# HarryShomer/LPFormer

Hardware: AMD Instinct MI355X
Metric: candidate link-pairs scored/sec (whole node) (higher is better)
Workload: dtype f32

## Files before the change

### lpformer_amd/csrc/tail_chain.hip

```cpp
#include <type_traits>

#include "lpf_common.h"

namespace {

typedef float f32x4 __attribute__((ext_vector_type(4)));

#ifndef LPF_TC_GROUPS
#define LPF_TC_GROUPS 4
#endif
constexpr int TC_GROUPS = LPF_TC_GROUPS;
constexpr int TC_WAVES = 2 * TC_GROUPS;
constexpr int TC_THREADS = 64 * TC_WAVES;

struct TailArgs {
    int64_t M;
    const float *x; int64_t ldx; int KA;
    const float *addend; int64_t ldadd;
    const float *wA, *lnA_g, *lnA_b; int NA;
    const float *tail; int64_t ldtail;
    const float *wB, *bB, *lnB_g, *lnB_b; int NB;
    const float *re; int64_t ldre;
    const float *wC, *bC; int NC;
    const float *wdot, *bdot;
    float *logit, *prob;
    const float *part;
    const float *bnd;
    int64_t units_cap;
    const int32_t *type_ptr;
    const float *att_bias;
    const int64_t *sel_ctl;
    int n_counts;
    const float *rows; int64_t ldrows;
    const int32_t *perm;
    const int64_t *n_full;
    const float *bC_empty;
    const float *row_empty;
    const float *X; int64_t ldX;
    const int64_t *batch; int64_t batch_ld, n_rows;
    const float *wE, *bE, *lnE_g, *lnE_b;
};

constexpr int tc_per_thread(int ntp) { return (ntp * 64 + TC_THREADS - 1) / TC_THREADS; }
constexpr int tc_stage_stride(int ntp) { return (ntp * 64 + 511) / 512 * 512; }

typedef short bf16x4_bits __attribute__((ext_vector_type(4)));
template <int P, int NTP, typename T>
__device__ __forceinline__ void tc_load(T (&r)[P], const float *packed, int stage, int tid) {
    const T *src = reinterpret_cast<const T *>(packed) + (int64_t)stage * tc_stage_stride(NTP);
#pragma unroll
    for (int e = 0; e < P; ++e) {
        const int i = e * TC_THREADS + tid;
#ifdef TC_NOWLOAD
        r[e] = T{};
        (void)src; (void)i;
#else
        r[e] = src[i < tc_stage_stride(NTP) ? i : 0];
#endif
    }
}
template <int P, typename T>
__device__ __forceinline__ void tc_store(const T (&r)[P], T *slab, int tid) {
#pragma unroll
    for (int e = 0; e < P; ++e) slab[e * TC_THREADS + tid] = r[e];
}

#define TC_PIN() __builtin_amdgcn_sched_barrier(0)

template <int TPW>
__device__ __forceinline__ void tc_mfma(f32x4 (&acc)[TPW], const f32x4 *lw, const f32x4 bv, bool last = true) {
    f32x4 a[TPW];
#pragma unroll
    for (int c = 0; c < TPW; ++c) a[c] = lw[c * 64];
#pragma unroll
    for (int u = 0; u < 4; ++u) {
#pragma unroll
        for (int c = 0; c < TPW - 1; ++c) acc[c] = __builtin_amdgcn_mfma_f32_16x16x4f32(a[c][u], bv[u], acc[c], 0, 0, 0);
        if (last) acc[TPW - 1] = __builtin_amdgcn_mfma_f32_16x16x4f32(a[TPW - 1][u], bv[u], acc[TPW - 1], 0, 0, 0);
    }
}
template <int TPW>
__device__ __forceinline__ void tc_mfma(f32x4 (&acc)[TPW], const uint2 *lw, const f32x4 bv, bool last = true) {
    bf16x4_bits b;
#pragma unroll
    for (int u = 0; u < 4; ++u) b[u] = (short)lpf_f32_to_bf16(bv[u]);
#pragma unroll
    for (int c = 0; c < TPW; ++c) {
        if (c == TPW - 1 && !last) break;
        const uint2 w = lw[c * 64];
        const bf16x4_bits a = {(short)(w.x & 0xffffu), (short)(w.x >> 16), (short)(w.y & 0xffffu), (short)(w.y >> 16)};
        acc[c] = __builtin_amdgcn_mfma_f32_16x16x16bf16_1k(a, b, acc[c], 0, 0, 0);
    }
}

constexpr int TC_XCH_SLOT = TC_WAVES * 16;
template <int TPW>
__device__ __forceinline__ void tc_layernorm(f32x4 (&acc)[TPW], int fbase, int n, const float *g, const float *b, int half,
                                             int q, float *my_x, const float *peer_x, bool relu) {
    float s1 = 0.f;
#pragma unroll
    for (int c = 0; c < TPW; ++c) s1 += acc[c][0] + acc[c][1] + acc[c][2] + acc[c][3];
    s1 = lpf_quad_sum(s1);
    if (q == 0) *my_x = s1;
    __syncthreads();
    const float mean = (half == 0 ? s1 + *peer_x : *peer_x + s1) / (float)n;
    float s2 = 0.f;
#pragma unroll
    for (int c = 0; c < TPW; ++c)
#pragma unroll
        for (int r = 0; r < 4; ++r) {
            const float d = (fbase + 16 * c + r < n) ? acc[c][r] - mean : 0.f;
            s2 += d * d;
        }
    s2 = lpf_quad_sum(s2);
    if (q == 0) my_x[TC_XCH_SLOT] = s2;
    __syncthreads();
    const float p2 = peer_x[TC_XCH_SLOT];
    const float rstd = 1.0f / sqrtf((half == 0 ? s2 + p2 : p2 + s2) / (float)n + 1e-5f);
#pragma unroll
    for (int c = 0; c < TPW; ++c) {
        const f32x4 gg = *reinterpret_cast<const f32x4 *>(g + fbase + 16 * c);
        const f32x4 bb = *reinterpret_cast<const f32x4 *>(b + fbase + 16 * c);
        acc[c] = (acc[c] - mean) * rstd * gg + bb;
        if (relu) {
#pragma unroll
            for (int r = 0; r < 4; ++r) acc[c][r] = fmaxf(acc[c][r], 0.f);
        }
    }
}

#ifdef TC_STAMPS
__device__ uint64_t *tc_stamp_buf = nullptr;
#define TC_STAMP(k) do { if (lane == 0) st_t[k] = wall_clock64(); } while (0)
#define TC_STAMPS_OUT(kind) do { if (lane == 0 && tc_stamp_buf) { uint64_t *o__ = tc_stamp_buf + ((int64_t)blockIdx.x * TC_WAVES + wave) * 16; \
        for (int k__ = 0; k__ < 10; ++k__) o__[k__] = st_t[k__]; o__[15] = (kind); } } while (0)
#define TC_STAMP_ROWS() do { __builtin_amdgcn_s_waitcnt(0x0f70); TC_STAMP(8); } while (0)
#else
#define TC_STAMP_ROWS() do { } while (0)
#define TC_STAMP(k) do { } while (0)
#define TC_STAMPS_OUT(kind) do { } while (0)
#endif

template <int NTA, int NTB, int NTC>
struct TcShape {
    static constexpr int NTPA = (NTA + 1) & ~1, NTPB = (NTB + 1) & ~1, NTPC = (NTC + 1) & ~1;
    static constexpr int PA = tc_per_thread(NTPA), PB = tc_per_thread(NTPB), PC = tc_per_thread(NTPC);
    static constexpr int PM = PA > PB ? (PA > PC ? PA : PC) : (PB > PC ? PB : PC);
    static constexpr int SLAB = PM * TC_THREADS;
    static constexpr int HT = NTPA > NTPB ? NTPA : NTPB;
    static constexpr int HID = TC_GROUPS * HT * 64;
    static constexpr int XCH = 5 * TC_WAVES * 16;
    static constexpr int VEC_B = 3 * 16 * NTPA, VEC_C = VEC_B + 3 * 16 * NTPB, VEC_N = VEC_C + 2 * 16 * NTPC;
    static constexpr size_t BYTES = (size_t)(2 * SLAB + HID) * sizeof(f32x4) + (XCH + VEC_N) * sizeof(float);
    static_assert(NTC >= 32 || BYTES <= 81920, "two workgroups share a CU's 160 KB of LDS");
};

template <int NTA, int NTB, int NTC, int WM = 0, bool ROWS = false, bool EW = false>
__global__ __launch_bounds__(TC_THREADS, NTC >= 32 ? 2 : (TC_THREADS >= 512 ? 4 : 3)) void tail_chain_kernel(const TailArgs A) {
    using S = TcShape<NTA, NTB, NTC>;
    constexpr bool WB = WM != 0;
    using WT = typename std::conditional<WM == 1, uint2, f32x4>::type;
    constexpr int NTPA = S::NTPA, NTPB = S::NTPB, NTPC = S::NTPC;
    constexpr int TPWA = NTPA / 2, TPWB = NTPB / 2, TPWC = NTPC / 2;
    constexpr int NGE = NTA;
    extern __shared__ __attribute__((aligned(16))) f32x4 lds[];
    f32x4 *hid = lds + 2 * S::SLAB;
    float *xch = reinterpret_cast<float *>(hid + S::HID);
    const int tid = threadIdx.x, lane = tid & 63, wave = tid >> 6;
    const int grp = wave >> 1, half = wave & 1, q = lane >> 4, j = lane & 15;
    float *my_x = xch + wave * 16 + j;
    const float *peer_x = xch + (wave ^ 1) * 16 + j;
    float *vec = xch + S::XCH;
    f32x4 *my_hid = hid + (grp * S::HT) * 64 + lane;
    int buf = 0;
#ifdef TC_STAMPS
    uint64_t st_t[10] = {0};
    TC_STAMP(0);
#endif

    const int64_t tile = blockIdx.x;
    const int64_t pos = tile * (16 * TC_GROUPS) + grp * 16 + j;
    const bool live = pos < A.M;
    bool lite = false;
    int64_t m = pos;
    if constexpr (ROWS) {
        if (A.perm) {
            m = A.perm[live ? pos : A.M - 1];
            lite = tile * (16 * TC_GROUPS) >= *A.n_full;
        }
    }
    const int64_t mm = live ? m : (ROWS && A.perm ? m : A.M - 1);
    bool no_sel = false;
    if constexpr (ROWS) no_sel = A.perm && A.row_empty && (live ? pos : A.M - 1) >= *A.n_full;

    constexpr int VP0 = EW ? 0 : S::VEC_B / 4, VPN = S::VEC_N / 4 - VP0, VPT = (VPN + TC_THREADS - 1) / TC_THREADS;
    f32x4 vecr[VPT];
#pragma unroll
    for (int e = 0; e < VPT; ++e) {
        int p = VP0 + e * TC_THREADS + tid;
        p = p < S::VEC_N / 4 ? p : S::VEC_N / 4 - 1;
        const float *src;
        if (p >= S::VEC_C / 4) {
            const int o = p - S::VEC_C / 4;
            src = o < 4 * NTPC ? (lite ? A.bC_empty : A.bC) + 4 * o : A.wdot + 4 * (o - 4 * NTPC);
        } else if (!EW || p >= S::VEC_B / 4) {
            const int o = p - S::VEC_B / 4;
            src = o < 4 * NTPB ? A.bB + 4 * o : (o < 8 * NTPB ? A.lnB_g + 4 * (o - 4 * NTPB) : A.lnB_b + 4 * (o - 8 * NTPB));
        } else {
            src = p < 4 * NTPA ? A.bE + 4 * p : (p < 8 * NTPA ? A.lnE_g + 4 * (p - 4 * NTPA) : A.lnE_b + 4 * (p - 8 * NTPA));
        }
        vecr[e] = *reinterpret_cast<const f32x4 *>(src);
    }
    TC_PIN();
    auto tc_vec_publish = [&]() __attribute__((always_inline)) {
#pragma unroll
        for (int e = 0; e < VPT; ++e) {
            int p = VP0 + e * TC_THREADS + tid;
            p = p < S::VEC_N / 4 ? p : S::VEC_N / 4 - 1;
            reinterpret_cast<f32x4 *>(vec)[p] = vecr[e];
        }
    };
    const float *v_bE = vec, *v_lnE_g = vec + 16 * NTPA, *v_lnE_b = vec + 32 * NTPA;
    const float *v_bB = vec + S::VEC_B, *v_lnB_g = v_bB + 16 * NTPB, *v_lnB_b = v_bB + 32 * NTPB;
    const float *v_bC = vec + S::VEC_C, *v_wdot = v_bC + 16 * NTPC;

    f32x4 rowv[ROWS ? TPWA : 1], rowt = (f32x4){0.f, 0.f, 0.f, 0.f};
#pragma unroll
    for (int c = 0; c < (ROWS ? TPWA : 1); ++c) rowv[c] = (f32x4){0.f, 0.f, 0.f, 0.f};
    auto tc_rows_request = [&]() __attribute__((always_inline)) {
        if constexpr (ROWS) {
            const int fbase = 16 * half * TPWA + 4 * q;
            const float *own = A.rows + mm * A.ldrows, *row = no_sel ? A.row_empty : own;
#pragma unroll
            for (int c = 0; c < TPWA; ++c) {
                const int f0 = fbase + 16 * c;
                rowv[c] = *reinterpret_cast<const f32x4 *>(row + (f0 < A.NA ? f0 : 0));
            }
            rowt = *reinterpret_cast<const f32x4 *>(own + A.NA);
        }
    };

    f32x4 accC[TPWC];
    if constexpr (EW) {
        static_assert(ROWS && WM == 0 && S::PA == 1 && NTPA == NTA && NGE % 2 == 0 && 2 * tc_stage_stride(NTPA) <= S::SLAB &&
                          tc_stage_stride(2 * NTPA) == 2 * tc_stage_stride(NTPA), "stage E: the fp32 rows form at D = 128");
        constexpr int TE_KG = 68, TE_Q2 = 34;
        static_assert((NGE - 1) * TE_KG + TE_Q2 + 32 <= S::HT * 64, "stage E's product tiles fit a group's hidden tiles");
        const int gj = 8 * half + (lane >> 3), gp = lane & 7;
        const int64_t gpos = tile * (16 * TC_GROUPS) + grp * 16 + gj;
        const int64_t gm = gpos < A.M ? gpos : A.M - 1;
        const int64_t gmm = A.perm ? A.perm[gm] : gm;
        int64_t ra = A.batch[gmm], rb = A.batch[A.batch_ld + gmm];
        WT wrE[2];
        tc_load<2, 2 * NTPA>(wrE, A.wE, 0, tid);
        TC_PIN();
        if ((uint64_t)ra >= (uint64_t)A.n_rows) ra = 0;
        if ((uint64_t)rb >= (uint64_t)A.n_rows) rb = 0;
        const float *xa = A.X + ra * A.ldX + 4 * gp, *xb = A.X + rb * A.ldX + 4 * gp;
        f32x4 accE[TPWA];
#pragma unroll
        for (int c = 0; c < TPWA; ++c) accE[c] = (f32x4){0.f, 0.f, 0.f, 0.f};
        f32x4 xra[NGE / 2], xrb[NGE / 2];
#pragma unroll
        for (int i = 0; i < NGE / 2; ++i) {
            xra[i] = *reinterpret_cast<const f32x4 *>(xa + 32 * i);
            xrb[i] = *reinterpret_cast<const f32x4 *>(xb + 32 * i);
        }
        tc_vec_publish();
        TC_STAMP_ROWS();
        {
            f32x4 *pe = hid + (grp * S::HT) * 64 + (gp >> 2) * TE_KG + ((gp >> 1) & 1) * TE_Q2 + (gp & 1) * 16 + gj;
#pragma unroll
            for (int i = 0; i < NGE / 2; ++i) pe[2 * i * TE_KG] = xra[i] * xrb[i];
        }
        const f32x4 *my_pe = hid + (grp * S::HT) * 64 + (q >> 1) * TE_Q2 + (q & 1) * 16 + j;
#pragma unroll
        for (int kg = 0; kg < NGE; kg += 2) {
            WT *lw = reinterpret_cast<WT *>(lds) + buf * S::SLAB;
            tc_store<2>(wrE, lw, tid);
            __syncthreads();
            if (kg + 2 < NGE) tc_load<2, 2 * NTPA>(wrE, A.wE, kg / 2 + 1, tid);
            TC_PIN();
            const f32x4 bv0 = my_pe[kg * TE_KG], bv1 = my_pe[(kg + 1) * TE_KG];
            tc_mfma<TPWA>(accE, lw + (half * TPWA) * 64 + lane, bv0);
            tc_mfma<TPWA>(accE, lw + tc_stage_stride(NTPA) + (half * TPWA) * 64 + lane, bv1);
            TC_PIN();
            buf ^= 1;
        }
        TC_STAMP(9);
        if (!lite) tc_rows_request();
        WT wrCe[S::PC];
        tc_load<S::PC, NTPC>(wrCe, A.wC, 0, tid);
        {
            const int fbase = 16 * half * TPWA + 4 * q;
#pragma unroll
            for (int c = 0; c < TPWA; ++c) accE[c] += *reinterpret_cast<const f32x4 *>(v_bE + fbase + 16 * c);
            tc_layernorm<TPWA>(accE, fbase, A.NA, v_lnE_g, v_lnE_b, half, q, my_x, peer_x, true);
#pragma unroll
            for (int c = 0; c < TPWA; ++c) my_hid[(half * TPWA + c) * 64] = accE[c];
        }
        TC_STAMP(7);
#pragma unroll
        for (int c = 0; c < TPWC; ++c) accC[c] = (f32x4){0.f, 0.f, 0.f, 0.f};
#pragma unroll 1
        for (int kg = 0; kg < NGE; ++kg) {
            WT *lw = reinterpret_cast<WT *>(lds) + buf * S::SLAB;
            tc_store<S::PC>(wrCe, lw, tid);
            __syncthreads();
            if (kg + 1 < NGE) tc_load<S::PC, NTPC>(wrCe, A.wC, kg + 1, tid);
            tc_mfma<TPWC>(accC, lw + (half * TPWC) * 64 + lane, my_hid[kg * 64]);
            buf ^= 1;
        }
        TC_STAMP(4);
        if (!lite) __syncthreads();
    }

    if constexpr (ROWS) {
        if (lite) {
            f32x4 (&acc)[TPWC] = accC;
            if constexpr (!EW) {
#pragma unroll
            for (int c = 0; c < TPWC; ++c) acc[c] = (f32x4){0.f, 0.f, 0.f, 0.f};
            WT wr[S::PC];
            const float *rer = A.re + mm * A.ldre + 4 * q;
            tc_load<S::PC, NTPC>(wr, A.wC, 0, tid);
            f32x4 xr = *reinterpret_cast<const f32x4 *>(rer);
            tc_vec_publish();
#pragma unroll 1
            for (int kg = 0; kg < NGE; ++kg) {
                const f32x4 bv = xr;
                WT *lw = reinterpret_cast<WT *>(lds) + buf * S::SLAB;
                tc_store<S::PC>(wr, lw, tid);
                __syncthreads();
                if (kg + 1 < NGE) {
                    tc_load<S::PC, NTPC>(wr, A.wC, kg + 1, tid);
                    xr = *reinterpret_cast<const f32x4 *>(rer + 16 * (kg + 1));
                }
                tc_mfma<TPWC>(acc, lw + (half * TPWC) * 64 + lane, bv);
                buf ^= 1;
            }
            }
            const int fbase = 16 * half * TPWC + 4 * q;
            float d = 0.f;
#pragma unroll
            for (int c = 0; c < TPWC; ++c) {
                const f32x4 b = *reinterpret_cast<const f32x4 *>(v_bC + fbase + 16 * c);
                const f32x4 w = *reinterpret_cast<const f32x4 *>(v_wdot + fbase + 16 * c);
#pragma unroll
                for (int r = 0; r < 4; ++r) d = fmaf(fmaxf(acc[c][r] + b[r], 0.f), w[r], d);
            }
            d = lpf_quad_sum(d);
            if (q == 0) my_x[4 * TC_XCH_SLOT] = d;
            __syncthreads();
            if (live && q == 0 && half == 0) {
                d = d + peer_x[4 * TC_XCH_SLOT] + A.bdot[0];
                if (A.sel_ctl && A.sel_ctl[3] != 0) d = __builtin_nanf("");
                if (A.logit) A.logit[m] = d;
                if (A.prob) A.prob[m] = 1.0f / (1.0f + expf(-d));
            }
            TC_STAMP(6);
            TC_STAMPS_OUT(1);
            return;
        }
    }
    if constexpr (!EW) tc_vec_publish();
    f32x4 accA[TPWA];
#pragma unroll
    for (int c = 0; c < TPWA; ++c) accA[c] = (f32x4){0.f, 0.f, 0.f, 0.f};
    int seg_cnt[3] = {0, 0, 0};
    if (!WB && !ROWS && A.part == nullptr) {
        const float *xa = A.x + mm * A.ldx;
        const int ngA = (A.KA + 15) >> 4;
        f32x4 wr[S::PA];
        tc_load<S::PA, NTPA>(wr, A.wA, 0, tid);
        int kk = 4 * q < A.KA ? 4 * q : A.KA - 4;
        f32x4 xr = *reinterpret_cast<const f32x4 *>(xa + kk);
#pragma unroll 1
        for (int kg = 0; kg < ngA; ++kg) {
            const f32x4 bv = (16 * kg + 4 * q < A.KA) ? xr : (f32x4){0.f, 0.f, 0.f, 0.f};
            f32x4 *lw = lds + buf * S::SLAB;
            tc_store<S::PA>(wr, lw, tid);
            __syncthreads();
            if (kg + 1 < ngA) {
                tc_load<S::PA, NTPA>(wr, A.wA, kg + 1, tid);
                kk = 16 * (kg + 1) + 4 * q;
                kk = kk < A.KA ? kk : A.KA - 4;
                xr = *reinterpret_cast<const f32x4 *>(xa + kk);
            }
            tc_mfma<TPWA>(accA, lw + (half * TPWA) * 64 + lane, bv);
            buf ^= 1;
        }
    }
    WT wrB[S::PB];
    tc_load<S::PB, NTPB>(wrB, A.wB, 0, tid);
    if constexpr (ROWS) {
        const int fbase = 16 * half * TPWA + 4 * q;
        if constexpr (!EW) tc_rows_request();
#pragma unroll
        for (int c = 0; c < TPWA; ++c) accA[c] = fbase + 16 * c < A.NA ? rowv[c] : (f32x4){0.f, 0.f, 0.f, 0.f};
    } else if (A.part == nullptr) {
        const int fbase = 16 * half * TPWA + 4 * q;
        f32x4 ad[TPWA];
#pragma unroll
        for (int c = 0; c < TPWA; ++c) {
            const int f0 = fbase + 16 * c;
            ad[c] = *reinterpret_cast<const f32x4 *>(A.addend + mm * A.ldadd + (f0 < A.NA ? f0 : 0));
        }
#pragma unroll
        for (int c = 0; c < TPWA; ++c) accA[c] += (fbase + 16 * c < A.NA) ? ad[c] : (f32x4){0.f, 0.f, 0.f, 0.f};
    } else {
        const int fbase = 16 * half * TPWA + 4 * q;
        const int64_t rs = A.NA + 4;
        float mx = -INFINITY, den = 0.f;
        f32x4 v[TPWA];
#pragma unroll
        for (int c = 0; c < TPWA; ++c) v[c] = (f32x4){0.f, 0.f, 0.f, 0.f};
        auto fetch = [&](const float *rec, f32x4 &h, f32x4 *b) __attribute__((always_inline)) {
            h = *reinterpret_cast<const f32x4 *>(rec + A.NA);
#pragma unroll
            for (int c = 0; c < TPWA; ++c) {
                const int f0 = fbase + 16 * c;
                b[c] = *reinterpret_cast<const f32x4 *>(rec + (f0 < A.NA ? f0 : 0));
            }
        };
        auto merge = [&](const f32x4 &h, const f32x4 *b) __attribute__((always_inline)) {
            const float mn = fmaxf(mx, h[0]);
            const float sa = __expf(mx - mn), sb = __expf(h[0] - mn);
            den = fmaf(den, sa, h[1] * sb);
#pragma unroll
            for (int c = 0; c < TPWA; ++c) v[c] = v[c] * sa + b[c] * sb;
            mx = mn;
        };
        int lo[3], hi[3], n_p[3];
#pragma unroll
        for (int t = 0; t < 3; ++t) {
            const int32_t *tp = A.type_ptr + (int64_t)t * (A.M + 1) + mm;
            lo[t] = tp[0];
            hi[t] = tp[1];
        }
        {
            f32x4 h0[3], b0[3][TPWA];
#pragma unroll
            for (int t = 0; t < 3; ++t) {
                seg_cnt[t] = hi[t] - lo[t];
                const bool some = hi[t] > lo[t] && ((hi[t] - 1) >> 4) < A.units_cap;
                n_p[t] = some ? ((hi[t] - 1) >> 4) - (lo[t] >> 4) + 1 : 0;
                const float *rec = n_p[t] > 1 ? A.bnd + ((((int64_t)t * A.units_cap + (lo[t] >> 4)) * 2) + 1) * rs
                                              : A.part + ((int64_t)t * A.M + mm) * rs;
                h0[t] = (f32x4){0.f, 0.f, 0.f, 0.f};
#pragma unroll
                for (int c = 0; c < TPWA; ++c) b0[t][c] = (f32x4){0.f, 0.f, 0.f, 0.f};
                if (n_p[t] > 0) fetch(rec, h0[t], b0[t]);
            }
#pragma unroll
            for (int t = 0; t < 3; ++t)
                if (n_p[t] > 0) merge(h0[t], b0[t]);
        }
        const int r0 = n_p[0] > 1 ? n_p[0] - 1 : 0, r1 = n_p[1] > 1 ? n_p[1] - 1 : 0, r2 = n_p[2] > 1 ? n_p[2] - 1 : 0;
        const int n_rest = r0 + r1 + r2;
        constexpr int NB = TPWA >= 4 ? 2 : 4;
#pragma unroll 1
        for (int k0 = 0; k0 < n_rest; k0 += NB) {
            f32x4 hh[NB], bb[NB][TPWA];
#pragma unroll
            for (int i = 0; i < NB; ++i) {
                const int k = k0 + i < n_rest ? k0 + i : n_rest - 1;
                const int t = k < r0 ? 0 : (k < r0 + r1 ? 1 : 2);
                const int jj = k - (t == 0 ? 0 : (t == 1 ? r0 : r0 + r1));
                const int ut = t == 0 ? lo[0] >> 4 : (t == 1 ? lo[1] >> 4 : lo[2] >> 4);
                fetch(A.bnd + (((int64_t)t * A.units_cap + ut + 1 + jj) * 2) * rs, hh[i], bb[i]);
            }
#pragma unroll
            for (int i = 0; i < NB; ++i)
                if (k0 + i < n_rest) merge(hh[i], bb[i]);
        }
        const float inv = 1.0f / (den + 1e-16f);
#pragma unroll
        for (int c = 0; c < TPWA; ++c) {
            const int f0 = fbase + 16 * c;
            if (f0 < A.NA) accA[c] = v[c] * inv + *reinterpret_cast<const f32x4 *>(A.att_bias + f0);
        }
    }
    {
        const int fbase = 16 * half * TPWA + 4 * q;
        if constexpr (!ROWS) tc_layernorm<TPWA>(accA, fbase, A.NA, A.lnA_g, A.lnA_b, half, q, my_x, peer_x, false);
#pragma unroll
        for (int c = 0; c < TPWA; ++c) my_hid[(half * TPWA + c) * 64] = accA[c];
    }

    TC_STAMP(1);
    f32x4 accB[TPWB];
#pragma unroll
    for (int c = 0; c < TPWB; ++c) accB[c] = (f32x4){0.f, 0.f, 0.f, 0.f};
    {
        f32x4 tailv = (f32x4){0.f, 0.f, 0.f, 0.f};
        if constexpr (ROWS) {
            if (q == 0 && !no_sel) tailv = rowt;
        } else if (q == 0) {
            if (A.part == nullptr) {
                tailv = *reinterpret_cast<const f32x4 *>(A.tail + mm * A.ldtail);
            } else {
                const float n0 = (float)seg_cnt[0], n1 = (float)seg_cnt[1], n2 = (float)seg_cnt[2];
                tailv = A.n_counts == 4 ? (f32x4){n0, n1, n2, n0 + n1}
                                         : (A.n_counts == 3 ? (f32x4){n0, n1, n0 + n1, 0.f} : (f32x4){n0, 0.f, 0.f, 0.f});
            }
        }
#pragma unroll
        for (int kg = 0; kg < NTPA + 1; ++kg) {
            WT *lw = reinterpret_cast<WT *>(lds) + buf * S::SLAB;
            tc_store<S::PB>(wrB, lw, tid);
            __syncthreads();
            if (kg + 1 < NTPA + 1) tc_load<S::PB, NTPB>(wrB, A.wB, kg + 1, tid);
            const f32x4 bv = kg < NTPA ? my_hid[(kg < NTPA ? kg : 0) * 64] : tailv;
            tc_mfma<TPWB>(accB, lw + (half * TPWB) * 64 + lane, bv, !((NTB & 1) && half == 1));
            buf ^= 1;
        }
    }
    TC_STAMP(2);
    WT wrC[S::PC];
    tc_load<S::PC, NTPC>(wrC, A.wC, EW ? NGE : 0, tid);
    const float *rer = EW ? nullptr : A.re + mm * A.ldre + 4 * q;
    f32x4 xr = (f32x4){0.f, 0.f, 0.f, 0.f};
    if constexpr (!EW) xr = *reinterpret_cast<const f32x4 *>(rer);
    {
        const int fbase = 16 * half * TPWB + 4 * q;
#pragma unroll
        for (int c = 0; c < TPWB; ++c) accB[c] += *reinterpret_cast<const f32x4 *>(v_bB + fbase + 16 * c);
        tc_layernorm<TPWB>(accB, fbase, A.NB, v_lnB_g, v_lnB_b, half, q, my_x + 2 * TC_XCH_SLOT, peer_x + 2 * TC_XCH_SLOT, true);
#pragma unroll
        for (int c = 0; c < TPWB; ++c) my_hid[(half * TPWB + c) * 64] = accB[c];
    }

    TC_STAMP(3);
    if constexpr (!EW) {
#pragma unroll
    for (int c = 0; c < TPWC; ++c) accC[c] = (f32x4){0.f, 0.f, 0.f, 0.f};
#pragma unroll 1
    for (int kg = 0; kg < NGE; ++kg) {
        const f32x4 bv = xr;
        WT *lw = reinterpret_cast<WT *>(lds) + buf * S::SLAB;
        tc_store<S::PC>(wrC, lw, tid);
        __syncthreads();
        tc_load<S::PC, NTPC>(wrC, A.wC, kg + 1, tid);
        if (kg + 1 < NGE) xr = *reinterpret_cast<const f32x4 *>(rer + 16 * (kg + 1));
        tc_mfma<TPWC>(accC, lw + (half * TPWC) * 64 + lane, bv);
        buf ^= 1;
    }
    TC_STAMP(4);
    }
#pragma unroll
    for (int kg = 0; kg < NTB; ++kg) {
        WT *lw = reinterpret_cast<WT *>(lds) + buf * S::SLAB;
        tc_store<S::PC>(wrC, lw, tid);
        __syncthreads();
        if (kg + 1 < NTB) tc_load<S::PC, NTPC>(wrC, A.wC, NGE + kg + 1, tid);
        TC_PIN();
        tc_mfma<TPWC>(accC, lw + (half * TPWC) * 64 + lane, my_hid[kg * 64]);
        TC_PIN();
        buf ^= 1;
    }
    TC_STAMP(5);
    {
        const int fbase = 16 * half * TPWC + 4 * q;
        float d = 0.f;
#pragma unroll
        for (int c = 0; c < TPWC; ++c) {
            const f32x4 b = *reinterpret_cast<const f32x4 *>(v_bC + fbase + 16 * c);
            const f32x4 w = *reinterpret_cast<const f32x4 *>(v_wdot + fbase + 16 * c);
#pragma unroll
            for (int r = 0; r < 4; ++r) d = fmaf(fmaxf(accC[c][r] + b[r], 0.f), w[r], d);
        }
        d = lpf_quad_sum(d);
        if (q == 0) my_x[4 * TC_XCH_SLOT] = d;
        __syncthreads();
        if (live && q == 0 && half == 0) {
            d = d + peer_x[4 * TC_XCH_SLOT] + A.bdot[0];
            if (A.sel_ctl && A.sel_ctl[3] != 0) d = __builtin_nanf("");
            if (A.logit) A.logit[m] = d;
            if (A.prob) A.prob[m] = 1.0f / (1.0f + expf(-d));
        }
    }
    TC_STAMP(6);
    TC_STAMPS_OUT(0);
}

template <int NTA, int NTB, int NTC, int WM = 0, bool ROWS = false, bool EW = false>
int tc_launch(const TailArgs &a, hipStream_t s) {
    constexpr size_t lds = TcShape<NTA, NTB, NTC>::BYTES;
    auto kern = tail_chain_kernel<NTA, NTB, NTC, WM, ROWS, EW>;
    LPF_SET_MAX_LDS(kern, lds);
    const int64_t blocks = (a.M + 16 * TC_GROUPS - 1) / (16 * TC_GROUPS);
    if (blocks > 0x7fffffff) return LPF_ERR_UNSUPPORTED;
    hipLaunchKernelGGL(kern, dim3((unsigned)blocks), dim3(TC_THREADS), lds, s, a);
    LPF_CHECK_LAUNCH();
    return LPF_OK;
}

}

#ifdef TC_STAMPS
extern "C" int lpf_tail_chain_set_stamps(void *buf) {
    return hipMemcpyToSymbol(HIP_SYMBOL(tc_stamp_buf), &buf, sizeof(buf)) == hipSuccess ? LPF_OK : LPF_ERR_LAUNCH;
}
#endif


extern "C" int lpf_tail_chain_f32(int64_t M, int32_t D, int32_t n_counts, const float *G, int64_t ldg,
                                  const float *wA_packed, const float *lnA_g, const float *lnA_b, const float *counts,
                                  int64_t ldc, const float *wB_packed, const float *bB, const float *lnB_g,
                                  const float *lnB_b, const float *r_e, int64_t ldre, const float *wC_packed,
                                  const float *bC, const float *w_dot, const float *b_dot, float *logit, float *prob,
                                  void *stream) {
    if (M == 0) return LPF_OK;
    LPF_REQUIRE(M > 0 && G && wA_packed && lnA_g && lnA_b && counts && wB_packed && bB && lnB_g && lnB_b && r_e &&
                wC_packed && bC && w_dot && b_dot && (logit || prob));
    LPF_REQUIRE(n_counts >= 1 && n_counts <= 4 && (ldg & 3) == 0 && ldg >= 4 * D + 4 && (ldc & 3) == 0 && ldc >= 4 &&
                (ldre & 3) == 0 && ldre >= D);
    LPF_REQUIRE(lpf_aligned16(G) && lpf_aligned16(counts) && lpf_aligned16(r_e) && lpf_aligned16(wA_packed) &&
                lpf_aligned16(wB_packed) && lpf_aligned16(wC_packed) && lpf_aligned16(lnA_g) && lpf_aligned16(lnA_b) &&
                lpf_aligned16(bB) && lpf_aligned16(lnB_g) && lpf_aligned16(lnB_b) && lpf_aligned16(bC) &&
                lpf_aligned16(w_dot));
    TailArgs a{M, G + D, ldg, 3 * D + 4, G, ldg, wA_packed, lnA_g, lnA_b, D, counts, ldc, wB_packed, bB, lnB_g,
               lnB_b, D + n_counts, r_e, ldre, wC_packed, bC, 2 * D, w_dot, b_dot, logit, prob,
               nullptr, nullptr, 0, nullptr, nullptr, nullptr, n_counts, nullptr, 0, nullptr, nullptr, nullptr, nullptr};
    hipStream_t s = static_cast<hipStream_t>(stream);
    switch (D) {
        case 32: return tc_launch<2, 3, 4>(a, s);
        case 64: return tc_launch<4, 5, 8>(a, s);
        case 128: return tc_launch<8, 9, 16>(a, s);
        default: return LPF_ERR_UNSUPPORTED;
    }
}

extern "C" int lpf_tail_chain_merge_f32(int64_t M, int32_t D, int32_t n_counts, const float *part, const float *bnd,
                                        int64_t units_cap, const int32_t *type_ptr, const float *att_bias, const float *lnA_g,
                                        const float *lnA_b, const float *wB_packed, const float *bB, const float *lnB_g,
                                        const float *lnB_b, const float *r_e, int64_t ldre, const float *wC_packed,
                                        const float *bC, const float *w_dot, const float *b_dot,
                                        const int64_t *sel_ctl, float *logit, float *prob, void *stream) {
    if (M == 0) return LPF_OK;
    LPF_REQUIRE(M > 0 && part && bnd && units_cap > 0 && lpf_aligned16(bnd) && type_ptr && att_bias && lnA_g && lnA_b && wB_packed && bB && lnB_g && lnB_b && r_e &&
                wC_packed && bC && w_dot && b_dot && (logit || prob));
    LPF_REQUIRE((n_counts == 1 || n_counts == 3 || n_counts == 4) && (ldre & 3) == 0 && ldre >= D);
    LPF_REQUIRE(lpf_aligned16(part) && lpf_aligned16(att_bias) && lpf_aligned16(r_e) && lpf_aligned16(wB_packed) &&
                lpf_aligned16(wC_packed) && lpf_aligned16(lnA_g) && lpf_aligned16(lnA_b) && lpf_aligned16(bB) &&
                lpf_aligned16(lnB_g) && lpf_aligned16(lnB_b) && lpf_aligned16(bC) && lpf_aligned16(w_dot));
    TailArgs a{M, nullptr, 0, 0, nullptr, 0, nullptr, lnA_g, lnA_b, D, nullptr, 0, wB_packed, bB, lnB_g,
               lnB_b, D + n_counts, r_e, ldre, wC_packed, bC, 2 * D, w_dot, b_dot, logit, prob,
               part, bnd, units_cap, type_ptr, att_bias, sel_ctl, n_counts, nullptr, 0, nullptr, nullptr, nullptr, nullptr};
    hipStream_t s = static_cast<hipStream_t>(stream);
    switch (D) {
        case 32: return tc_launch<2, 3, 4>(a, s);
        case 64: return tc_launch<4, 5, 8>(a, s);
        case 128: return tc_launch<8, 9, 16>(a, s);
        default: return LPF_ERR_UNSUPPORTED;
    }
}

extern "C" int lpf_tail_chain_merge_bf16(int64_t M, int32_t D, int32_t n_counts, const float *part, const float *bnd,
                                         int64_t units_cap, const int32_t *type_ptr, const float *att_bias,
                                         const float *lnA_g, const float *lnA_b, const void *wB_packed_bf16,
                                         const float *bB, const float *lnB_g, const float *lnB_b, const float *r_e,
                                         int64_t ldre, const void *wC_packed_bf16, const float *bC, const float *w_dot,
                                         const float *b_dot, const int64_t *sel_ctl, float *logit, float *prob,
                                         void *stream) {
    if (M == 0) return LPF_OK;
    LPF_REQUIRE(M > 0 && part && bnd && units_cap > 0 && lpf_aligned16(bnd) && type_ptr && att_bias && lnA_g && lnA_b &&
                wB_packed_bf16 && bB && lnB_g && lnB_b && r_e && wC_packed_bf16 && bC && w_dot && b_dot &&
                (logit || prob));
    LPF_REQUIRE((n_counts == 1 || n_counts == 3 || n_counts == 4) && (ldre & 3) == 0 && ldre >= D);
    LPF_REQUIRE(lpf_aligned16(part) && lpf_aligned16(att_bias) && lpf_aligned16(r_e) && lpf_aligned16(wB_packed_bf16) &&
                lpf_aligned16(wC_packed_bf16) && lpf_aligned16(lnA_g) && lpf_aligned16(lnA_b) && lpf_aligned16(bB) &&
                lpf_aligned16(lnB_g) && lpf_aligned16(lnB_b) && lpf_aligned16(bC) && lpf_aligned16(w_dot));
    TailArgs a{M, nullptr, 0, 0, nullptr, 0, nullptr, lnA_g, lnA_b, D, nullptr, 0,
               static_cast<const float *>(wB_packed_bf16), bB, lnB_g, lnB_b, D + n_counts, r_e, ldre,
               static_cast<const float *>(wC_packed_bf16), bC, 2 * D, w_dot, b_dot, logit, prob,
               part, bnd, units_cap, type_ptr, att_bias, sel_ctl, n_counts, nullptr, 0, nullptr, nullptr, nullptr, nullptr};
    hipStream_t s = static_cast<hipStream_t>(stream);
    switch (D) {
        case 32: return tc_launch<2, 3, 4, 1>(a, s);
        case 64: return tc_launch<4, 5, 8, 1>(a, s);
        case 128: return tc_launch<8, 9, 16, 1>(a, s);
        default: return LPF_ERR_UNSUPPORTED;
    }
}

namespace {
template <int WM>
int tc_rows(int64_t M, int32_t D, int32_t n_counts, const float *rows, int64_t ldrows, const void *wB, const float *bB,
            const float *lnB_g, const float *lnB_b, const float *r_e, int64_t ldre, const void *wC, const float *bC,
            const float *w_dot, const float *b_dot, const int64_t *sel_ctl, float *logit, float *prob, void *stream,
            const int32_t *perm = nullptr, const int64_t *n_full = nullptr, const float *bC_empty = nullptr,
            const float *row_empty = nullptr) {
    if (M == 0) return LPF_OK;
    LPF_REQUIRE(!perm || (n_full && bC_empty && lpf_aligned16(bC_empty)));
    LPF_REQUIRE(!row_empty || (perm && lpf_aligned16(row_empty)));
    LPF_REQUIRE(M > 0 && rows && wB && bB && lnB_g && lnB_b && r_e && wC && bC && w_dot && b_dot && (logit || prob));
    LPF_REQUIRE((n_counts == 1 || n_counts == 3 || n_counts == 4) && (ldre & 3) == 0 && ldre >= D && (ldrows & 3) == 0 &&
                ldrows >= D + 4);
    LPF_REQUIRE(lpf_aligned16(rows) && lpf_aligned16(r_e) && lpf_aligned16(wB) && lpf_aligned16(wC) && lpf_aligned16(bB) &&
                lpf_aligned16(lnB_g) && lpf_aligned16(lnB_b) && lpf_aligned16(bC) && lpf_aligned16(w_dot));
    TailArgs a{M, nullptr, 0, 0, nullptr, 0, nullptr, nullptr, nullptr, D, nullptr, 0, static_cast<const float *>(wB), bB,
               lnB_g, lnB_b, D + n_counts, r_e, ldre, static_cast<const float *>(wC), bC, 2 * D, w_dot, b_dot, logit, prob,
               nullptr, nullptr, 0, nullptr, nullptr, sel_ctl, n_counts, rows, ldrows, perm, n_full, bC_empty, row_empty};
    hipStream_t s = static_cast<hipStream_t>(stream);
    switch (D) {
        case 32: return tc_launch<2, 3, 4, WM, true>(a, s);
        case 64: return tc_launch<4, 5, 8, WM, true>(a, s);
        case 128: return tc_launch<8, 9, 16, WM, true>(a, s);
        case 256: return tc_launch<16, 17, 32, WM, true>(a, s);
        default: return LPF_ERR_UNSUPPORTED;
    }
}
// ... 73 lines not shown
```

Measured before the change: 282.1 million.

## Software-pipeline weight staging across all tail-chain GEMM stages with shared register buffer

Restructures every k-group loop in the tail chain kernel so the next weight stage is stored to the alternate LDS slab and the stage after is fetched from global memory while the current MFMAs run. This removes one of the two barriers per k-group by putting the store inside the MFMA sequence. A single shared register stage replaces the per-stage buffers, which lets the last loads of one GEMM prefetch the first weights of the next stage across stage boundaries. The cost is more complex compile-time unrolled control flow, a raw s_waitcnt, and a risk of higher register pressure or correctness bugs at stage seams.

```diff
diff --git a/lpformer_amd/csrc/tail_chain.hip b/lpformer_amd/csrc/tail_chain.hip
--- a/lpformer_amd/csrc/tail_chain.hip
+++ b/lpformer_amd/csrc/tail_chain.hip
@@ -1,4 +1,5 @@
 #include <type_traits>
+#include <utility>
 
 #include "lpf_common.h"
 
@@ -45,8 +46,9 @@
 constexpr int tc_stage_stride(int ntp) { return (ntp * 64 + 511) / 512 * 512; }
 
 typedef short bf16x4_bits __attribute__((ext_vector_type(4)));
-template <int P, int NTP, typename T>
-__device__ __forceinline__ void tc_load(T (&r)[P], const float *packed, int stage, int tid) {
+template <int P, int NTP, int PM, typename T>
+__device__ __forceinline__ void tc_load(T (&r)[PM], const float *packed, int stage, int tid) {
+    static_assert(P <= PM, "the register stage holds a weight stage");
     const T *src = reinterpret_cast<const T *>(packed) + (int64_t)stage * tc_stage_stride(NTP);
 #pragma unroll
     for (int e = 0; e < P; ++e) {
@@ -59,37 +61,73 @@
 #endif
     }
 }
-template <int P, typename T>
-__device__ __forceinline__ void tc_store(const T (&r)[P], T *slab, int tid) {
+template <int P, int PM, typename T>
+__device__ __forceinline__ void tc_store(const T (&r)[PM], T *slab, int tid) {
+    static_assert(P <= PM, "the register stage holds a weight stage");
 #pragma unroll
     for (int e = 0; e < P; ++e) slab[e * TC_THREADS + tid] = r[e];
 }
 
 #define TC_PIN() __builtin_amdgcn_sched_barrier(0)
-
-template <int TPW>
-__device__ __forceinline__ void tc_mfma(f32x4 (&acc)[TPW], const f32x4 *lw, const f32x4 bv, bool last = true) {
-    f32x4 a[TPW];
-#pragma unroll
-    for (int c = 0; c < TPW; ++c) a[c] = lw[c * 64];
-#pragma unroll
-    for (int u = 0; u < 4; ++u) {
-#pragma unroll
-        for (int c = 0; c < TPW - 1; ++c) acc[c] = __builtin_amdgcn_mfma_f32_16x16x4f32(a[c][u], bv[u], acc[c], 0, 0, 0);
-        if (last) acc[TPW - 1] = __builtin_amdgcn_mfma_f32_16x16x4f32(a[TPW - 1][u], bv[u], acc[TPW - 1], 0, 0, 0);
-    }
-}
-template <int TPW>
-__device__ __forceinline__ void tc_mfma(f32x4 (&acc)[TPW], const uint2 *lw, const f32x4 bv, bool last = true) {
+struct TcNoStep { __device__ __forceinline__ void operator()() const {} };
+__device__ __forceinline__ void tc_kgroup_barrier() { __syncthreads(); }
+template <int STEP, typename F, int... I>
+__device__ __forceinline__ void tc_each_impl(F &f, std::integer_sequence<int, I...>) {
+    (f(std::integral_constant<int, I * STEP>()), ...);
+}
+template <int N, int STEP = 1, typename F>
+__device__ __forceinline__ void tc_each(F f) {
+    tc_each_impl<STEP>(f, std::make_integer_sequence<int, (N + STEP - 1) / STEP>());
+}
+
+template <int TPW, typename Step = TcNoStep>
+__device__ __forceinline__ void tc_mfma(f32x4 (&acc)[TPW], const f32x4 *lw, const f32x4 bv, bool last = true,
+                                        Step step = Step()) {
+    constexpr int H = TPW >= 8 ? 4 : TPW;
+#pragma unroll
+    for (int h = 0; h < TPW; h += H) {
+        f32x4 a[H];
+#pragma unroll
+        for (int c = 0; c < H; ++c) a[c] = lw[(h + c < TPW ? h + c : TPW - 1) * 64];
+#pragma unroll
+        for (int u = 0; u < 4; ++u) {
+            if (h + H >= TPW && last)
+                acc[TPW - 1] = __builtin_amdgcn_mfma_f32_16x16x4f32(a[TPW - 1 - h][u], bv[u], acc[TPW - 1], 0, 0, 0);
+#pragma unroll
+            for (int c = 0; c < H; ++c)
+                if (h + c < TPW - 1) acc[h + c] = __builtin_amdgcn_mfma_f32_16x16x4f32(a[c][u], bv[u], acc[h + c], 0, 0, 0);
+            if constexpr (!std::is_same<Step, TcNoStep>::value) {
+                if (u == 0 && h == 0) {
+                    TC_PIN();
+                    step();
+                    TC_PIN();
+                }
+            }
+        }
+    }
+}
+template <int TPW, typename Step = TcNoStep>
+__device__ __forceinline__ void tc_mfma(f32x4 (&acc)[TPW], const uint2 *lw, const f32x4 bv, bool last = true,
+                                        Step step = Step()) {
     bf16x4_bits b;
 #pragma unroll
     for (int u = 0; u < 4; ++u) b[u] = (short)lpf_f32_to_bf16(bv[u]);
+    uint2 w[TPW];
+#pragma unroll
+    for (int c = 0; c < TPW; ++c) w[c] = lw[c * 64];
 #pragma unroll
     for (int c = 0; c < TPW; ++c) {
         if (c == TPW - 1 && !last) break;
-        const uint2 w = lw[c * 64];
-        const bf16x4_bits a = {(short)(w.x & 0xffffu), (short)(w.x >> 16), (short)(w.y & 0xffffu), (short)(w.y >> 16)};
+        const bf16x4_bits a = {(short)(w[c].x & 0xffffu), (short)(w[c].x >> 16), (short)(w[c].y & 0xffffu),
+                               (short)(w[c].y >> 16)};
         acc[c] = __builtin_amdgcn_mfma_f32_16x16x16bf16_1k(a, b, acc[c], 0, 0, 0);
+        if constexpr (!std::is_same<Step, TcNoStep>::value) {
+            if (c == 0) {
+                TC_PIN();
+                step();
+                TC_PIN();
+            }
+        }
     }
 }
 
@@ -173,6 +211,8 @@
     float *vec = xch + S::XCH;
     f32x4 *my_hid = hid + (grp * S::HT) * 64 + lane;
     int buf = 0;
+    WT wr[S::PM];
+    WT *const slabs = reinterpret_cast<WT *>(lds);
 #ifdef TC_STAMPS
     uint64_t st_t[10] = {0};
     TC_STAMP(0);
@@ -230,7 +270,7 @@
     auto tc_rows_request = [&]() __attribute__((always_inline)) {
         if constexpr (ROWS) {
             const int fbase = 16 * half * TPWA + 4 * q;
-            const float *own = A.rows + mm * A.ldrows, *row = no_sel ? A.row_empty : own;
+            const float *own = A.rows + (EW && lite ? 0 : mm * A.ldrows), *row = no_sel ? A.row_empty : own;
 #pragma unroll
             for (int c = 0; c < TPWA; ++c) {
                 const int f0 = fbase + 16 * c;
@@ -251,8 +291,8 @@
         const int64_t gm = gpos < A.M ? gpos : A.M - 1;
         const int64_t gmm = A.perm ? A.perm[gm] : gm;
         int64_t ra = A.batch[gmm], rb = A.batch[A.batch_ld + gmm];
-        WT wrE[2];
-        tc_load<2, 2 * NTPA>(wrE, A.wE, 0, tid);
+        static_assert(S::PM >= 2 && S::PC <= S::PM && NGE >= 4, "stage E's weight stages fit the register stage");
+        tc_load<2, 2 * NTPA>(wr, A.wE, 0, tid);
         TC_PIN();
         if ((uint64_t)ra >= (uint64_t)A.n_rows) ra = 0;
         if ((uint64_t)rb >= (uint64_t)A.n_rows) rb = 0;
@@ -266,6 +306,9 @@
             xra[i] = *reinterpret_cast<const f32x4 *>(xa + 32 * i);
             xrb[i] = *reinterpret_cast<const f32x4 *>(xb + 32 * i);
         }
+        tc_store<2>(wr, slabs + buf * S::SLAB, tid);
+        tc_load<2, 2 * NTPA>(wr, A.wE, 1, tid);
+        TC_PIN();
         tc_vec_publish();
         TC_STAMP_ROWS();
         {
@@ -274,23 +317,26 @@
             for (int i = 0; i < NGE / 2; ++i) pe[2 * i * TE_KG] = xra[i] * xrb[i];
         }
         const f32x4 *my_pe = hid + (grp * S::HT) * 64 + (q >> 1) * TE_Q2 + (q & 1) * 16 + j;
-#pragma unroll
-        for (int kg = 0; kg < NGE; kg += 2) {
-            WT *lw = reinterpret_cast<WT *>(lds) + buf * S::SLAB;
-            tc_store<2>(wrE, lw, tid);
-            __syncthreads();
-            if (kg + 2 < NGE) tc_load<2, 2 * NTPA>(wrE, A.wE, kg / 2 + 1, tid);
-            TC_PIN();
+        __syncthreads();
+        tc_each<NGE, 2>([&](auto KG) __attribute__((always_inline)) {
+            constexpr int kg = decltype(KG)::value;
+            const WT *lw = slabs + buf * S::SLAB;
+            WT *nw = slabs + (buf ^ 1) * S::SLAB;
             const f32x4 bv0 = my_pe[kg * TE_KG], bv1 = my_pe[(kg + 1) * TE_KG];
-            tc_mfma<TPWA>(accE, lw + (half * TPWA) * 64 + lane, bv0);
+            tc_mfma<TPWA>(accE, lw + (half * TPWA) * 64 + lane, bv0, true, [&]() __attribute__((always_inline)) {
+                if constexpr (kg + 2 < NGE) tc_store<2>(wr, nw, tid);
+                else tc_store<S::PC>(wr, nw, tid);
+                if constexpr (kg + 4 < NGE) tc_load<2, 2 * NTPA>(wr, A.wE, kg / 2 + 2, tid);
+                else tc_load<S::PC, NTPC>(wr, A.wC, (kg + 4 - NGE) / 2, tid);
+            });
             tc_mfma<TPWA>(accE, lw + tc_stage_stride(NTPA) + (half * TPWA) * 64 + lane, bv1);
             TC_PIN();
             buf ^= 1;
-        }
+            if constexpr (kg + 2 < NGE) tc_kgroup_barrier();
+        });
         TC_STAMP(9);
-        if (!lite) tc_rows_request();
-        WT wrCe[S::PC];
-        tc_load<S::PC, NTPC>(wrCe, A.wC, 0, tid);
+        tc_rows_request();
+        TC_PIN();
         {
             const int fbase = 16 * half * TPWA + 4 * q;
 #pragma unroll
@@ -302,17 +348,30 @@
         TC_STAMP(7);
 #pragma unroll
         for (int c = 0; c < TPWC; ++c) accC[c] = (f32x4){0.f, 0.f, 0.f, 0.f};
-#pragma unroll 1
-        for (int kg = 0; kg < NGE; ++kg) {
-            WT *lw = reinterpret_cast<WT *>(lds) + buf * S::SLAB;
-            tc_store<S::PC>(wrCe, lw, tid);
-            __syncthreads();
-            if (kg + 1 < NGE) tc_load<S::PC, NTPC>(wrCe, A.wC, kg + 1, tid);
-            tc_mfma<TPWC>(accC, lw + (half * TPWC) * 64 + lane, my_hid[kg * 64]);
+        __syncthreads();
+        tc_each<NGE>([&](auto KG) __attribute__((always_inline)) {
+            constexpr int kg = decltype(KG)::value;
+            const WT *lw = slabs + buf * S::SLAB;
+            WT *nw = slabs + (buf ^ 1) * S::SLAB;
+            tc_mfma<TPWC>(accC, lw + (half * TPWC) * 64 + lane, my_hid[kg * 64], true, [&]() __attribute__((always_inline)) {
+                if constexpr (kg + 2 < NGE) {
+                    tc_store<S::PC>(wr, nw, tid);
+                    tc_load<S::PC, NTPC>(wr, A.wC, kg + 2, tid);
+                } else if (!lite) {
+                    if constexpr (kg + 1 < NGE) tc_store<S::PC>(wr, nw, tid);
+                    else tc_store<S::PB>(wr, nw, tid);
+                    if constexpr (kg + 2 == NGE) tc_load<S::PB, NTPB>(wr, A.wB, 0, tid);
+                    else tc_load<S::PB, NTPB>(wr, A.wB, 1, tid);
+                } else if constexpr (kg + 1 < NGE) {
+                    tc_store<S::PC>(wr, nw, tid);
+                }
+            });
+            TC_PIN();
             buf ^= 1;
-        }
+            if constexpr (kg + 1 < NGE) tc_kgroup_barrier();
+            else if (!lite) __syncthreads();
+        });
         TC_STAMP(4);
-        if (!lite) __syncthreads();
     }
 
     if constexpr (ROWS) {
@@ -321,23 +380,40 @@
             if constexpr (!EW) {
 #pragma unroll
             for (int c = 0; c < TPWC; ++c) acc[c] = (f32x4){0.f, 0.f, 0.f, 0.f};
-            WT wr[S::PC];
+            static_assert(NGE >= 2, "the stream's start requests two stages");
             const float *rer = A.re + mm * A.ldre + 4 * q;
             tc_load<S::PC, NTPC>(wr, A.wC, 0, tid);
-            f32x4 xr = *reinterpret_cast<const f32x4 *>(rer);
+            f32x4 x0 = *reinterpret_cast<const f32x4 *>(rer), x1 = (f32x4){0.f, 0.f, 0.f, 0.f};
             tc_vec_publish();
+            tc_store<S::PC>(wr, slabs + buf * S::SLAB, tid);
+            tc_load<S::PC, NTPC>(wr, A.wC, 1, tid);
+            TC_PIN();
+            __syncthreads();
+            auto group = [&](int kg, const f32x4 &xc, f32x4 &xn) __attribute__((always_inline)) {
+                const WT *lw = slabs + buf * S::SLAB;
+                WT *nw = slabs + (buf ^ 1) * S::SLAB;
+                tc_mfma<TPWC>(acc, lw + (half * TPWC) * 64 + lane, xc, true, [&]() __attribute__((always_inline)) {
+                    tc_store<S::PC>(wr, nw, tid);
+                    xn = *reinterpret_cast<const f32x4 *>(rer + 16 * (kg + 1 < NGE ? kg + 1 : NGE - 1));
+                    tc_load<S::PC, NTPC>(wr, A.wC, kg + 2 < NGE ? kg + 2 : NGE - 1, tid);
+                });
+                TC_PIN();
+                buf ^= 1;
+                if (kg + 1 < NGE) tc_kgroup_barrier();
+            };
+            static_assert(NGE % 2 == 0, "k-groups in pairs");
+            if constexpr (NGE == 8) {
+#pragma unroll
+                for (int kg = 0; kg < NGE; kg += 2) {
+                    group(kg, x0, x1);
+                    group(kg + 1, x1, x0);
+                }
+            } else {
 #pragma unroll 1
-            for (int kg = 0; kg < NGE; ++kg) {
-                const f32x4 bv = xr;
-                WT *lw = reinterpret_cast<WT *>(lds) + buf * S::SLAB;
-                tc_store<S::PC>(wr, lw, tid);
-                __syncthreads();
-                if (kg + 1 < NGE) {
-                    tc_load<S::PC, NTPC>(wr, A.wC, kg + 1, tid);
-                    xr = *reinterpret_cast<const f32x4 *>(rer + 16 * (kg + 1));
+                for (int kg = 0; kg < NGE; kg += 2) {
+                    group(kg, x0, x1);
+                    group(kg + 1, x1, x0);
                 }
-                tc_mfma<TPWC>(acc, lw + (half * TPWC) * 64 + lane, bv);
-                buf ^= 1;
             }
             }
             const int fbase = 16 * half * TPWC + 4 * q;
@@ -368,34 +444,61 @@
 #pragma unroll
     for (int c = 0; c < TPWA; ++c) accA[c] = (f32x4){0.f, 0.f, 0.f, 0.f};
     int seg_cnt[3] = {0, 0, 0};
-    if (!WB && !ROWS && A.part == nullptr) {
+    const bool gemmA = !WB && !ROWS && A.part == nullptr;
+    if constexpr (!WB && !ROWS) {
+    if (gemmA) {
         const float *xa = A.x + mm * A.ldx;
         const int ngA = (A.KA + 15) >> 4;
-        f32x4 wr[S::PA];
         tc_load<S::PA, NTPA>(wr, A.wA, 0, tid);
         int kk = 4 * q < A.KA ? 4 * q : A.KA - 4;
         f32x4 xr = *reinterpret_cast<const f32x4 *>(xa + kk);
-#pragma unroll 1
-        for (int kg = 0; kg < ngA; ++kg) {
-            const f32x4 bv = (16 * kg + 4 * q < A.KA) ? xr : (f32x4){0.f, 0.f, 0.f, 0.f};
-            f32x4 *lw = lds + buf * S::SLAB;
-            tc_store<S::PA>(wr, lw, tid);
-            __syncthreads();
-            if (kg + 1 < ngA) {
-                tc_load<S::PA, NTPA>(wr, A.wA, kg + 1, tid);
+        tc_store<S::PA>(wr, slabs + buf * S::SLAB, tid);
+        if (ngA > 1) tc_load<S::PA, NTPA>(wr, A.wA, 1, tid);
+        else tc_load<S::PB, NTPB>(wr, A.wB, 0, tid);
+        TC_PIN();
+        __syncthreads();
+        f32x4 x1 = (f32x4){0.f, 0.f, 0.f, 0.f};
+        auto group = [&](int kg, const f32x4 &xc, f32x4 &xn) __attribute__((always_inline)) {
+            const f32x4 bv = (16 * kg + 4 * q < A.KA) ? xc : (f32x4){0.f, 0.f, 0.f, 0.f};
+            const f32x4 *lw = slabs + buf * S::SLAB;
+            f32x4 *nw = slabs + (buf ^ 1) * S::SLAB;
+            tc_mfma<TPWA>(accA, lw + (half * TPWA) * 64 + lane, bv, true, [&]() __attribute__((always_inline)) {
+                if (kg + 1 < ngA) tc_store<S::PA>(wr, nw, tid);
+                else tc_store<S::PB>(wr, nw, tid);
                 kk = 16 * (kg + 1) + 4 * q;
                 kk = kk < A.KA ? kk : A.KA - 4;
-                xr = *reinterpret_cast<const f32x4 *>(xa + kk);
-            }
-            tc_mfma<TPWA>(accA, lw + (half * TPWA) * 64 + lane, bv);
+                xn = *reinterpret_cast<const f32x4 *>(xa + kk);
+                if (kg + 2 < ngA) tc_load<S::PA, NTPA>(wr, A.wA, kg + 2, tid);
+                else tc_load<S::PB, NTPB>(wr, A.wB, kg + 2 - ngA, tid);
+            });
+            TC_PIN();
             buf ^= 1;
-        }
-    }
-    WT wrB[S::PB];
-    tc_load<S::PB, NTPB>(wrB, A.wB, 0, tid);
+            tc_kgroup_barrier();
+        };
+        int kg = 0;
+#pragma unroll 1
+        for (; kg + 1 < ngA; kg += 2) {
+            group(kg, xr, x1);
+            group(kg + 1, x1, xr);
+        }
+        if (kg < ngA) group(kg, xr, x1);
+    }
+    }
+    if constexpr (!EW) {
+        if (!gemmA) tc_load<S::PB, NTPB>(wr, A.wB, 0, tid);
+    }
+    auto tc_b_start = [&]() __attribute__((always_inline)) {
+        tc_store<S::PB>(wr, slabs + buf * S::SLAB, tid);
+        tc_load<S::PB, NTPB>(wr, A.wB, 1, tid);
+        TC_PIN();
+    };
     if constexpr (ROWS) {
         const int fbase = 16 * half * TPWA + 4 * q;
-        if constexpr (!EW) tc_rows_request();
+        if constexpr (!EW) {
+            tc_rows_request();
+            TC_PIN();
+            tc_b_start();
+        }
 #pragma unroll
         for (int c = 0; c < TPWA; ++c) accA[c] = fbase + 16 * c < A.NA ? rowv[c] : (f32x4){0.f, 0.f, 0.f, 0.f};
     } else if (A.part == nullptr) {
@@ -483,7 +586,10 @@
     }
     {
         const int fbase = 16 * half * TPWA + 4 * q;
-        if constexpr (!ROWS) tc_layernorm<TPWA>(accA, fbase, A.NA, A.lnA_g, A.lnA_b, half, q, my_x, peer_x, false);
+        if constexpr (!ROWS) {
+            if (!gemmA) tc_b_start();
+            tc_layernorm<TPWA>(accA, fbase, A.NA, A.lnA_g, A.lnA_b, half, q, my_x, peer_x, false);
+        }
 #pragma unroll
         for (int c = 0; c < TPWA; ++c) my_hid[(half * TPWA + c) * 64] = accA[c];
     }
@@ -492,6 +598,8 @@
     f32x4 accB[TPWB];
 #pragma unroll
     for (int c = 0; c < TPWB; ++c) accB[c] = (f32x4){0.f, 0.f, 0.f, 0.f};
+    const float *rer = EW ? nullptr : A.re + mm * A.ldre + 4 * q;
+    f32x4 xr = (f32x4){0.f, 0.f, 0.f, 0.f};
     {
         f32x4 tailv = (f32x4){0.f, 0.f, 0.f, 0.f};
         if constexpr (ROWS) {
@@ -505,22 +613,31 @@
                                          : (A.n_counts == 3 ? (f32x4){n0, n1, n0 + n1, 0.f} : (f32x4){n0, 0.f, 0.f, 0.f});
             }
         }
-#pragma unroll
-        for (int kg = 0; kg < NTPA + 1; ++kg) {
-            WT *lw = reinterpret_cast<WT *>(lds) + buf * S::SLAB;
-            tc_store<S::PB>(wrB, lw, tid);
-            __syncthreads();
-            if (kg + 1 < NTPA + 1) tc_load<S::PB, NTPB>(wrB, A.wB, kg + 1, tid);
+        constexpr int NKB = NTPA + 1;
+        constexpr int C0 = EW ? NGE : 0;
+        static_assert(NKB >= 2 && NTB >= 2, "a stage's last two weight steps are the next stage's first two");
+        __syncthreads();
+        tc_each<NKB>([&](auto KG) __attribute__((always_inline)) {
+            constexpr int kg = decltype(KG)::value;
+            const WT *lw = slabs + buf * S::SLAB;
+            WT *nw = slabs + (buf ^ 1) * S::SLAB;
             const f32x4 bv = kg < NTPA ? my_hid[(kg < NTPA ? kg : 0) * 64] : tailv;
-            tc_mfma<TPWB>(accB, lw + (half * TPWB) * 64 + lane, bv, !((NTB & 1) && half == 1));
+            tc_mfma<TPWB>(accB, lw + (half * TPWB) * 64 + lane, bv, !((NTB & 1) && half == 1),
+                          [&]() __attribute__((always_inline)) {
+                if constexpr (kg + 1 < NKB) tc_store<S::PB>(wr, nw, tid);
+                else tc_store<S::PC>(wr, nw, tid);
+                if constexpr (kg + 2 < NKB) tc_load<S::PB, NTPB>(wr, A.wB, kg + 2, tid);
+                else {
+                    if constexpr (kg + 2 == NKB) tc_load<S::PC, NTPC>(wr, A.wC, C0, tid);
+                    else tc_load<S::PC, NTPC>(wr, A.wC, C0 + 1, tid);
+                }
+            });
+            TC_PIN();
             buf ^= 1;
-        }
+            if constexpr (kg + 1 < NKB) tc_kgroup_barrier();
+        });
     }
     TC_STAMP(2);
-    WT wrC[S::PC];
-    tc_load<S::PC, NTPC>(wrC, A.wC, EW ? NGE : 0, tid);
-    const float *rer = EW ? nullptr : A.re + mm * A.ldre + 4 * q;
-    f32x4 xr = (f32x4){0.f, 0.f, 0.f, 0.f};
     if constexpr (!EW) xr = *reinterpret_cast<const f32x4 *>(rer);
     {
         const int fbase = 16 * half * TPWB + 4 * q;
@@ -532,33 +649,52 @@
     }
 
     TC_STAMP(3);
+    __syncthreads();
     if constexpr (!EW) {
 #pragma unroll
     for (int c = 0; c < TPWC; ++c) accC[c] = (f32x4){0.f, 0.f, 0.f, 0.f};
-#pragma unroll 1
-    for (int kg = 0; kg < NGE; ++kg) {
-        const f32x4 bv = xr;
-        WT *lw = reinterpret_cast<WT *>(lds) + buf * S::SLAB;
-        tc_store<S::PC>(wrC, lw, tid);
-        __syncthreads();
-        tc_load<S::PC, NTPC>(wrC, A.wC, kg + 1, tid);
-        if (kg + 1 < NGE) xr = *reinterpret_cast<const f32x4 *>(rer + 16 * (kg + 1));
-        tc_mfma<TPWC>(accC, lw + (half * TPWC) * 64 + lane, bv);
-        buf ^= 1;
-    }
-    TC_STAMP(4);
-    }
-#pragma unroll
-    for (int kg = 0; kg < NTB; ++kg) {
-        WT *lw = reinterpret_cast<WT *>(lds) + buf * S::SLAB;
-        tc_store<S::PC>(wrC, lw, tid);
-        __syncthreads();
-        if (kg + 1 < NTB) tc_load<S::PC, NTPC>(wrC, A.wC, NGE + kg + 1, tid);
-        TC_PIN();
-        tc_mfma<TPWC>(accC, lw + (half * TPWC) * 64 + lane, my_hid[kg * 64]);
+    __builtin_amdgcn_s_waitcnt(0x0f70);
+    f32x4 x1 = (f32x4){0.f, 0.f, 0.f, 0.f};
+    auto group = [&](int kg, const f32x4 &xc, f32x4 &xn) __attribute__((always_inline)) {
+        const WT *lw = slabs + buf * S::SLAB;
+        WT *nw = slabs + (buf ^ 1) * S::SLAB;
+        tc_mfma<TPWC>(accC, lw + (half * TPWC) * 64 + lane, xc, true, [&]() __attribute__((always_inline)) {
+            tc_store<S::PC>(wr, nw, tid);
+            xn = *reinterpret_cast<const f32x4 *>(rer + 16 * (kg + 1 < NGE ? kg + 1 : NGE - 1));
+            tc_load<S::PC, NTPC>(wr, A.wC, kg + 2, tid);
+        });
         TC_PIN();
         buf ^= 1;
-    }
+        tc_kgroup_barrier();
+    };
+    static_assert(NGE % 2 == 0, "k-groups in pairs");
+    if constexpr (NGE == 8) {
+#pragma unroll
+        for (int kg = 0; kg < NGE; kg += 2) {
+            group(kg, xr, x1);
+            group(kg + 1, x1, xr);
+        }
+    } else {
+#pragma unroll 1
+        for (int kg = 0; kg < NGE; kg += 2) {
+            group(kg, xr, x1);
+            group(kg + 1, x1, xr);
+        }
+    }
+    TC_STAMP(4);
+    }
+    tc_each<NTB>([&](auto KG) __attribute__((always_inline)) {
+        constexpr int kg = decltype(KG)::value;
+        const WT *lw = slabs + buf * S::SLAB;
+        WT *nw = slabs + (buf ^ 1) * S::SLAB;
+        tc_mfma<TPWC>(accC, lw + (half * TPWC) * 64 + lane, my_hid[kg * 64], true, [&]() __attribute__((always_inline)) {
+            if constexpr (kg + 1 < NTB) tc_store<S::PC>(wr, nw, tid);
+            if constexpr (kg + 2 < NTB) tc_load<S::PC, NTPC>(wr, A.wC, NGE + kg + 2, tid);
+        });
+        TC_PIN();
+        buf ^= 1;
+        if constexpr (kg + 1 < NTB) tc_kgroup_barrier();
+    });
     TC_STAMP(5);
     {
         const int fbase = 16 * half * TPWC + 4 * q;
```

New measurement: 286.2 million, median of 6. +1.5%, better.
